# ku222/Attention-GAN

Hardware: AMD Instinct MI355X
Metric: train images/sec at 256×256 stage-3, batch 24/GPU, 1/2/4/8 MI355X (higher is better)
Workload: dtype f32; 1 GPU; full 3-stage AttnGAN 64->128->256 train step: G + 3xD updates + word attention + DAMSM words/sentence loss + KL + 4x fused Adam (BASELINE.json configs[2]); workload_key=full3, batch_per_gpu=24, global_batch=24, gf_dim=32, df_dim=64, emb_dim=256, seq_len=10, text_encoder=bypassed (frozen; N(0,1) embeddings), parallelism=dp1, discriminator_streams=3, launch=eager, gradient_exchange=none (one rank), losses_finite=True

## Files before the change

attention-gan_amd/backend/functional.py:

```python
from __future__ import annotations

import ctypes
import math
from ctypes import byref, c_void_p
from typing import Dict, Optional, Tuple

import contextlib
import os
import weakref

import torch
from torch import Tensor
from torch.autograd import Function
from torch.autograd.function import once_differentiable

from . import lib as L

_PRECISION = [L.PREC_F32]


def set_precision(p: int) -> None:
    if int(p) != _PRECISION[0]:
        for rng in _FLAT_RANGES:
            rng[3], rng[4] = [], None
# ... 418 lines not shown
        return
    cur = torch.cuda.current_stream()
    key = cur.cuda_stream
    if _SIDE_DIRTY.get(key):
        cur.wait_stream(_SIDE_STREAMS[key])
        _SIDE_DIRTY[key] = False


class ActHandoff:
    __slots__ = ("masked",)

    def __init__(self):
        self.masked = False


class _ConvFn(Function):
    @staticmethod
    def forward(ctx, x: Tensor, weight: Tensor, bias: Optional[Tensor], kind: str, cache: Optional[dict], wdst, bdst, act: int = 0,
                handoff_out: Optional[ActHandoff] = None, handoff_in: Optional[ActHandoff] = None):
        x = _act(x, "conv input")
        w = _dev(weight.detach(), "conv weight")
        B, Cin, H, W = x.shape
        Cout, Cin_w, kh, kw = w.shape
        if Cin != Cin_w or kh != kw:
            raise L.AganError(f"conv: input has {Cin} channels, weight {tuple(w.shape)}")
        gf, pf, gd, pd, (OH, OW) = conv_geoms(kind, B, Cin, H, W, Cout, kh)
        pe = effective_precision(gf)
        x, odt = _gather_types(gf, pe, x, get_activation_storage())
        out = torch.empty((B, Cout, OH, OW), dtype=_TORCH_OF[odt], device=x.device)
        b = _dev(bias.detach(), "conv bias") if bias is not None else None
        need_xs = pe == L.PREC_F16X3 or (ctx.needs_input_grad[1] and _needs_amax() and wgrad_effective_precision(gf, pf) == L.PREC_F16X3)
        xs = amax_of(x) if need_xs else None
        _gather(x, packed_weight(w, pf, cache, pe), b, gf, out, kind, "fwd", act, None, pe, xs)
        ctx.x_scale = xs
        if act == L.ACT_NONE:
            ctx.save_for_backward(x, w)
        else:
            ctx.save_for_backward(x, w, out)
        ctx.kind, ctx.has_bias, ctx.cache, ctx.wdst, ctx.bdst, ctx.act = kind, bias is not None, cache, wdst, bdst, act
        ctx.handoff_out = handoff_out if act != L.ACT_NONE else None
        ctx.handoff_in = handoff_in if (handoff_in is not None and Cin > 4) else None
        return out

    @staticmethod
    @once_differentiable
    def backward(ctx, dy: Tensor):
        x, w = ctx.saved_tensors[:2]
        dy = _act(dy, "conv grad")
# ... 43 lines not shown
                if obs is not None:
                    obs.end()
            if want_b:
                dbbuf, bacc, db = _grad_out(ctx.bdst, (Cout,), x)
                L.call("agan_bias_grad", _p(_dev(dy, "conv grad")), _p(dbbuf), B, Cout, dy.shape[2] * dy.shape[3], bacc, _stream())
        if ctx.needs_input_grad[0]:
            dyg, ddt = _gather_types(gd, pe_d, dy, _dt(x))
            dx = torch.empty(x.shape, dtype=_TORCH_OF[ddt], device=x.device)
            mask = x if ctx.handoff_in is not None else None
            if mask is not None and mask.dtype != dx.dtype:
                mask = mask.to(dx.dtype)
            _gather(dyg, packed_weight(w, pd, ctx.cache, pe_d), None, gd, dx, ctx.kind, "dgrad", L.ACT_NONE, mask, pe_d,
                    dys if pe_d == L.PREC_F16X3 else None)
            if mask is not None:
                ctx.handoff_in.masked = True
        return dx, dw, db, None, None, None, None, None, None, None


def conv_fuses_activation(act: int, cout: int) -> bool:
    return act == L.ACT_LRELU and cout > 4


def conv2d(x: Tensor, weight: Tensor, bias: Optional[Tensor] = None, kind: str = "same", cache: Optional[dict] = None,
           wdst=None, bdst=None, act: int = 0, handoff_out: Optional[ActHandoff] = None,
           handoff_in: Optional[ActHandoff] = None) -> Tensor:
    return _ConvFn.apply(x, weight, bias, kind, cache, wdst, bdst, act, handoff_out, handoff_in)


def linear(x: Tensor, weight: Tensor, bias: Optional[Tensor] = None, cache: Optional[dict] = None, wdst=None, bdst=None) -> Tensor:
    B, Cin = x.shape
    y = _ConvFn.apply(x.reshape(B, Cin, 1, 1), weight.view(weight.shape[0], Cin, 1, 1), bias, "same", cache, wdst, bdst)
    return y.view(B, weight.shape[0])


_BN_GROUPS = [1]


@contextlib.contextmanager
def bn_groups(groups: int):
    old = _BN_GROUPS[0]
    _BN_GROUPS[0] = int(groups)
    try:
        yield
    finally:
        _BN_GROUPS[0] = old


class _BnActFn(Function):
    @staticmethod
    def forward(ctx, x, gamma, beta, residual, running_mean, running_var, nbt, training, act, eps, momentum, gdst, bdst, groups):
        x = _act(x, "bn input")
        shape = x.shape
        B, C = shape[0], shape[1]
        HW = x.numel() // (B * C)
        if not training:
            groups = 1
        if B % groups:
            raise L.AganError(f"BatchNorm: batch {B} does not split into {groups} groups")
        Bg = B // groups
        g, b = _dev(gamma.detach(), "bn weight"), _dev(beta.detach(), "bn bias")
        lib = L.load()
        co = C // 2 if act == L.ACT_GLU else C
        odt = get_activation_storage() if HW > 1 else L.DT_F32
        if x.dtype != torch.float32 and _dt(x) != odt:
            x = x.float()
        xdt = _dt(x)
        out = torch.empty((B, co) + tuple(shape[2:]), dtype=_TORCH_OF[odt], device=x.device)
        res = _act(residual, "bn residual") if residual is not None else None
        if res is not None and res.dtype != out.dtype:
            res = res.to(out.dtype)
        if training:
            mean = torch.empty((groups, C), dtype=torch.float32, device=x.device)
            invstd = torch.empty_like(mean)
            nbytes = lib.agan_bn_train_fwd_ws_bytes(Bg, C, HW)
            ws, wsp = _ws(nbytes, x)
            L.call("agan_bn_train_fwd_dt", _p(x), _p(g), _p(b), _p(res), _p(out), _p(mean), _p(invstd), _p(running_mean),
                   _p(running_var), _p(nbt), B, C, HW, float(eps), float(momentum), act, groups, wsp, nbytes, _stream(),
                   _p(_amax_out(out)), xdt, odt)
        else:
            mean = running_mean
            invstd = torch.rsqrt(running_var + eps)
            L.call("agan_bn_act_fwd_dt", _p(x), _p(mean), _p(invstd), _p(g), _p(b), _p(res), _p(out), B, C, HW, act, _stream(),
                   _p(_amax_out(out)), xdt, odt)
        ctx.save_for_backward(x, g, b, mean, invstd)
        ctx.odt = odt
        ctx.act, ctx.training, ctx.has_res, ctx.gdst, ctx.bdst, ctx.groups = act, training, residual is not None, gdst, bdst, groups
        return out

    @staticmethod
    @once_differentiable
    def backward(ctx, dout):
        if not ctx.training:
            raise L.AganError("BatchNorm backward in eval mode is not on the training path")
# ... 3 lines not shown
            dout = dout.to(_TORCH_OF[ctx.odt])
        B, C = x.shape[0], x.shape[1]
        HW = x.numel() // (B * C)
        groups = ctx.groups
        Bg = B // groups
        dx = torch.empty_like(x)
        dgbuf, gacc, dg = _grad_out(ctx.gdst if ctx.needs_input_grad[1] else None, g.shape, x)
        dbbuf, bacc, db = _grad_out(ctx.bdst if ctx.needs_input_grad[2] else None, b.shape, x)
        if gacc != bacc:
            raise L.AganError("BatchNorm weight/bias gradient destinations out of step")
        nbytes = L.load().agan_bn_act_bwd_ws_bytes(Bg, C, HW)
        ws, wsp = _ws(nbytes, x)
        L.call("agan_bn_act_bwd_dt", _p(x), _p(dout), _p(mean), _p(invstd), _p(g), _p(b), _p(dx), _p(dgbuf), _p(dbbuf), B, C, HW,
               ctx.act, gacc, groups, wsp, nbytes, _stream(), _p(_amax_out(dx)), _dt(x), ctx.odt)
        dres = dout if ctx.has_res else None
        return dx, dg, db, dres, None, None, None, None, None, None, None, None, None, None


def bn_act(x, gamma, beta, running_mean, running_var, nbt, training: bool, act: int, residual=None,
           eps: float = 1e-5, momentum: float = 0.1) -> Tensor:
    return _BnActFn.apply(x, gamma, beta, residual, running_mean, running_var, nbt, training, act, eps, momentum,
                          grad_dst(gamma), grad_dst(beta), _BN_GROUPS[0])


class _ActFn(Function):
    @staticmethod
    def forward(ctx, x, act):
        x = _dev(x, "activation input")
        out = torch.empty_like(x)
        L.call("agan_act_fwd", _p(x), _p(out), x.numel(), act, _stream())
        ctx.save_for_backward(out)
        ctx.act = act
        return out

    @staticmethod
    @once_differentiable
    def backward(ctx, dout):
# ... 688 lines not shown
```

attention-gan_amd/backend/lib.py:

```python
from __future__ import annotations

import ctypes
import os
from ctypes import POINTER, Structure, c_char_p, c_double, c_float, c_int, c_int32, c_int64, c_size_t, c_void_p

_HERE = os.path.dirname(os.path.abspath(__file__))
LIB_PATH = os.environ.get("AGAN_LIB") or os.path.join(os.path.dirname(_HERE), "csrc", "libagan_hip.so")

PREC_F32, PREC_BF16, PREC_BF16X3, PREC_F16, PREC_BF16X6, PREC_F16X3 = 0, 1, 2, 3, 4, 5
PRECISIONS = {"f32": PREC_F32, "bf16": PREC_BF16, "bf16x3": PREC_BF16X3, "f16": PREC_F16, "bf16x6": PREC_BF16X6, "f16x3": PREC_F16X3}
PACK_FWD, PACK_DGRAD_S1, PACK_DGRAD_4x4S2, PACK_UP_FWD, PACK_UP_DGRAD, PACK_DGRAD_3x3S2 = 0, 1, 2, 3, 4, 5
ACT_NONE, ACT_GLU, ACT_LRELU, ACT_TANH, ACT_SIGMOID, ACT_RELU = 0, 1, 2, 3, 4, 5
COMM_ID_BYTES = 128
DT_F32, DT_BF16, DT_F16 = 0, 1, 2
AMAX_SLOT = 256
ABI_VERSION = 101


class ConvGeom(Structure):
    _fields_ = [("B", c_int32), ("Cin", c_int32), ("IH", c_int32), ("IW", c_int32),
                ("Cout", c_int32), ("OH", c_int32), ("OW", c_int32), ("R", c_int32), ("S", c_int32),
                ("OS", c_int32), ("SY", c_int32), ("DY", c_int32), ("OY", c_int32 * 2)]


# ... 30 lines not shown
    "agan_pack_weight": (c_int, [_P, _P, c_int, c_int, c_int, c_int, c_int, c_int, _P]),
    "agan_conv_effective_prec": (c_int, [POINTER(ConvGeom), c_int]),
    "agan_conv_wgrad_effective_prec": (c_int, [POINTER(ConvGeom), c_int, c_int]),
    "agan_conv_executed_fraction": (c_double, [POINTER(ConvGeom), c_int, c_int, c_int]),
    "agan_conv_gather_ws_bytes": (c_size_t, [POINTER(ConvGeom), c_int]),
    "agan_conv_ktable_elems": (c_size_t, [POINTER(ConvGeom)]),
    "agan_conv_ktable": (c_int, [POINTER(ConvGeom), _P, _P]),
    "agan_conv_gather": (c_int, [_P, _P, _P, _P, POINTER(ConvGeom), _P, c_int, c_int, _P, _P, c_size_t, _P, _P, _P]),
    "agan_conv_gather_dt": (c_int, [_P, _P, _P, _P, POINTER(ConvGeom), _P, c_int, c_int, _P, _P, c_size_t, _P, _P, _P, c_int, c_int]),
    "agan_conv_gather_dt_supported": (c_int, [POINTER(ConvGeom), c_int, c_int, c_int]),
    "agan_conv_wgrad_dt_supported": (c_int, [POINTER(ConvGeom), c_int, c_int, c_int, c_int]),
    "agan_conv_wgrad_dt": (c_int, [_P, _P, _P, POINTER(ConvGeom), _P, c_int, c_int, c_int, c_int, c_int, _P, c_size_t, _P, _P, _P, c_int, c_int]),
    "agan_bn_stats_dt": (c_int, [_P, c_int, c_int, c_int, c_float, _P, _P, _P, _P, _P, c_float, _P, c_size_t, _P, c_int]),
    "agan_bn_act_fwd_dt": (c_int, [_P, _P, _P, _P, _P, _P, _P, c_int, c_int, c_int, c_int, _P, _P, c_int, c_int]),
    "agan_bn_train_fwd_dt": (c_int, [_P, _P, _P, _P, _P, _P, _P, _P, _P, _P, c_int, c_int, c_int, c_float, c_float, c_int, c_int, _P, c_size_t, _P, _P, c_int, c_int]),
    "agan_bn_act_bwd_dt": (c_int, [_P, _P, _P, _P, _P, _P, _P, _P, _P, c_int, c_int, c_int, c_int, c_int, c_int, _P, c_size_t, _P, _P, c_int, c_int]),
    "agan_absmax": (c_int, [_P, c_size_t, _P, _P]),
    "agan_conv_wgrad_ws_bytes": (c_size_t, [POINTER(ConvGeom)]),
    "agan_conv_wgrad": (c_int, [_P, _P, _P, POINTER(ConvGeom), _P, c_int, c_int, c_int, c_int, c_int, _P, c_size_t, _P, _P, _P]),
    "agan_bias_grad": (c_int, [_P, _P, c_int, c_int, c_int, c_int, _P]),
    "agan_bn_stats_ws_bytes": (c_size_t, [c_int, c_int, c_int]),
    "agan_bn_stats": (c_int, [_P, c_int, c_int, c_int, c_float, _P, _P, _P, _P, _P, c_float, _P, c_size_t, _P]),
    "agan_bn_train_fwd_ws_bytes": (c_size_t, [c_int, c_int, c_int]),
    "agan_bn_train_fwd": (c_int, [_P] * 10 + [c_int, c_int, c_int, c_float, c_float, c_int, c_int, _P, c_size_t, _P, _P]),
    "agan_bn_act_fwd": (c_int, [_P, _P, _P, _P, _P, _P, _P, c_int, c_int, c_int, c_int, _P, _P]),
    "agan_bn_act_bwd_ws_bytes": (c_size_t, [c_int, c_int, c_int]),
    "agan_bn_act_bwd": (c_int, [_P] * 9 + [c_int, c_int, c_int, c_int, c_int, c_int, _P, c_size_t, _P, _P]),
    "agan_act_fwd": (c_int, [_P, _P, c_size_t, c_int, _P]),
    "agan_act_bwd": (c_int, [_P, _P, _P, c_size_t, c_int, _P]),
    "agan_glu_fwd": (c_int, [_P, _P, c_int, c_int, c_int, _P]),
# ... 84 lines not shown
```

attention-gan_amd/csrc/agan_common.h:

```cpp
#pragma once
#include <hip/hip_runtime.h>
#include <stdint.h>
#include <stdio.h>
#include <string.h>

#include "../../include/agan.h"

namespace agan {

constexpr int kWave = 64;

void set_error(const char* fmt, ...);

#define AGAN_REQUIRE(cond, ...)            \
    do {                                    \
        if (!(cond)) {                      \
            agan::set_error(__VA_ARGS__);   \
            return AGAN_EINVAL;             \
        }                                   \
    } while (0)

inline int check_launch(const char* what) {
    hipError_t e = hipGetLastError();
    if (e != hipSuccess) {
// ... 158 lines not shown
}

template <int NT>
__device__ __forceinline__ float block_sum(float v, float* smem) {
    v = wave_sum(v);
    const int w = threadIdx.x >> 6;
    __syncthreads();
    if ((threadIdx.x & 63) == 0) smem[w] = v;
    __syncthreads();
    float r = 0.f;
#pragma unroll
    for (int i = 0; i < NT / 64; ++i) r += smem[i];
    return r;
}

}
```

attention-gan_amd/csrc/bn_act.hip:

```cpp
#include "agan_common.h"

#include <algorithm>
#include <type_traits>

using namespace agan;

namespace {

constexpr float kSlope = 0.2f;

__device__ __forceinline__ float sigmoidf_(float v) { return 1.f / (1.f + __expf(-v)); }

__host__ __device__ __forceinline__ int vec_width(bool any16, int HW) { return (any16 && (HW & 7) == 0) ? 8 : ((HW & 3) == 0 ? 4 : 1); }

constexpr int kLogCap = 64;
thread_local int g_log[kLogCap];
thread_local int g_log_n = 0;
enum { kLogStatsPartial = 1, kLogStatsFinal, kLogStatsRows, kLogFwdApply, kLogSmallFwd, kLogSmallBwd, kLogBwdPartial, kLogBwdFinal,
       kLogBwdApply, kLogActFwd, kLogActBwd, kLogGluFwd, kLogGluBwd };
inline void log_reset() { g_log_n = 0; }
inline void log_launch(int kind, int act, int xdt, int odt, int width) {
    if (g_log_n < kLogCap) g_log[g_log_n] = kind * 100000 + act * 10000 + xdt * 1000 + odt * 100 + width;
    ++g_log_n;
}

struct Chunk { int beg, end; };

__device__ __forceinline__ Chunk chunk_of(int n, int nchunk, int chunk) {
    int len = (cdiv(n, nchunk) + 7) & ~7;
    Chunk c;
    c.beg = min(n, chunk * len);
    c.end = min(n, c.beg + len);
    return c;
}
// ... 355 lines not shown

constexpr int kSmallN = 8192;
constexpr int kSmallPer = kSmallN / 256;

__device__ __forceinline__ void block_sum2_d(double& a, double& b, double (*red)[4]) {
    a = wave_sum_d(a);
    b = wave_sum_d(b);
    const int w = threadIdx.x >> 6;
    __syncthreads();
    if ((threadIdx.x & 63) == 0) { red[0][w] = a; red[1][w] = b; }
    __syncthreads();
    a = red[0][0] + red[0][1] + red[0][2] + red[0][3];
    b = red[1][0] + red[1][1] + red[1][2] + red[1][3];
}

template <int ACT, int XDT, int ODT, int PER = kSmallPer>
__global__ __launch_bounds__(256) void bn_small_fwd_kernel(const void* __restrict__ x, const float* __restrict__ gamma, const float* __restrict__ beta,
                                                           const void* __restrict__ res, void* __restrict__ out, float* __restrict__ mean,
                                                           float* __restrict__ invstd, float* __restrict__ rmean, float* __restrict__ rvar,
                                                           int64_t* __restrict__ nbt, int B, int C, int HW, float eps, float momentum,
                                                           float* __restrict__ amax) {
    __shared__ double red[2][4];
    constexpr bool GLU = ACT == AGAN_ACT_GLU;
    const int Co = GLU ? C / 2 : C;
    const int c = blockIdx.x, n = B * HW;
    if (c == 0 && threadIdx.x == 0 && nbt) *nbt += 1;
    float va[PER], vg[GLU ? PER : 1];
    double s = 0.0, q = 0.0, sg = 0.0, qg = 0.0;
#pragma unroll
    for (int j = 0; j < PER; ++j) {
        const int i = threadIdx.x + j * 256;
        va[j] = 0.f;
        if (GLU) vg[j] = 0.f;
        if (i < n) {
            const int b = i / HW, p = i - b * HW;
            const size_t xi = ((size_t)b * C + c) * HW + p;
            va[j] = ld1<XDT>(x, xi);
            s += va[j];
            q += (double)va[j] * va[j];
            if (GLU) {
                vg[j] = ld1<XDT>(x, xi + (size_t)Co * HW);
                sg += vg[j];
                qg += (double)vg[j] * vg[j];
            }
        }
    }
    block_sum2_d(s, q, red);
    const double m = s / n;
    double var = q / n - m * m;
    var = var < 0.0 ? 0.0 : var;
    const float is = (float)(1.0 / sqrt(var + (double)eps));
    float mgf = 0.f, isg = 0.f;
    double mg = 0.0, varg = 0.0;
    if (GLU) {
        block_sum2_d(sg, qg, red);
        mg = sg / n;
// ... 9 lines not shown
        if (rmean) {
            rmean[c] = (float)((1.0 - momentum) * rmean[c] + momentum * m);
            rvar[c] = (float)((1.0 - momentum) * rvar[c] + momentum * var * ub);
        }
        if (GLU) {
            mean[c + Co] = mgf;
            invstd[c + Co] = isg;
            if (rmean) {
                rmean[c + Co] = (float)((1.0 - momentum) * rmean[c + Co] + momentum * mg);
                rvar[c + Co] = (float)((1.0 - momentum) * rvar[c + Co] + momentum * varg * ub);
            }
        }
    }
    const Affine a = make_affine((float)m, is, gamma[c], beta[c]);
    const Affine g = GLU ? make_affine(mgf, isg, gamma[c + Co], beta[c + Co]) : a;
    float mx = 0.f;
#pragma unroll
    for (int j = 0; j < PER; ++j) {
        const int i = threadIdx.x + j * 256;
        if (i < n) {
            const int b = i / HW, p = i - b * HW;
            const size_t oi = ((size_t)b * Co + c) * HW + p;
            float z = norm_of(a, va[j]);
            if (GLU) z *= sigmoidf_(norm_of(g, vg[j]));
            else if (ACT == AGAN_ACT_LRELU) z = z > 0.f ? z : z * kSlope;
            if (!GLU && ACT == AGAN_ACT_NONE && res) z += ld1<ODT>(res, oi);
            st1<ODT>(out, oi, z);
            mx = fmaxf(mx, fabsf(z));
        }
    }
    if (amax) amax_commit(mx, amax);
}

template <int ACT, int XDT, int ODT, int PER = kSmallPer>
__global__ __launch_bounds__(256) void bn_small_bwd_kernel(const void* __restrict__ x, const void* __restrict__ dout, const float* __restrict__ mean,
                                                           const float* __restrict__ invstd, const float* __restrict__ gamma,
                                                           const float* __restrict__ beta, void* __restrict__ dx, float* __restrict__ dgamma,
                                                           float* __restrict__ dbeta, int B, int C, int HW, int accumulate,
                                                           float* __restrict__ amax) {
    __shared__ double red[2][4];
    constexpr bool GLU = ACT == AGAN_ACT_GLU;
    const int Co = GLU ? C / 2 : C;
    const int c = blockIdx.x, n = B * HW;
    const Affine a = affine_of(mean, invstd, gamma, beta, c);
// ... 352 lines not shown
        if (int e = bn_stats_impl(xg, Bg, C, HW, eps, mg, ig, running_mean, running_var, nbt, momentum, ws, ws_bytes, stream, x_dtype)) return e;
        if (int e = bn_act_fwd_impl(xg, mg, ig, gamma, beta, residual ? off(residual, (size_t)gi * Bg * Co * HW, out_dtype) : nullptr,
                                       off(out, (size_t)gi * Bg * Co * HW, out_dtype), Bg, C, HW, act, stream, out_amax, x_dtype, out_dtype))
            return e;
    }
    return AGAN_OK;
}
int agan_bn_train_fwd(const float* x, const float* gamma, const float* beta, const float* residual, float* out, float* mean,
                      float* invstd, float* running_mean, float* running_var, int64_t* nbt, int B, int C, int HW, float eps,
                      float momentum, int act, int groups, void* ws, size_t ws_bytes, void* stream, float* out_amax) {
    return agan_bn_train_fwd_dt(x, gamma, beta, residual, out, mean, invstd, running_mean, running_var, nbt, B, C, HW, eps, momentum, act,
                                groups, ws, ws_bytes, stream, out_amax, AGAN_DT_F32, AGAN_DT_F32);
}

}
```

attention-gan_amd/csrc/conv.hip:

```cpp
#include "conv_common.h"

#include <cxxabi.h>
#include <cstdlib>


using namespace agan;

using namespace agan::conv;

namespace {

__global__ __launch_bounds__(256) void ktable_kernel(int2* __restrict__ tab, int n, int K, int RS, int S, int IHW, int IW, int DY) {
    const int k = blockIdx.x * 256 + threadIdx.x;
    if (k >= n) return;
    int2 a, b;
    if (k < K) {
        const int c = k / RS, rs = k - c * RS, r = rs / S, q = rs - r * S;
        const int dy = r * DY, dx = q * DY;
        a.x = c * IHW + dy * IW + dx;
        a.y = (dy & 0xFFFF) | (dx << 16);
        b.x = c * IHW * 4;
        b.y = rs * kTapRowBytes;
    } else {
        a.x = 0;
// ... 1053 lines not shown

int agan_conv_ktable(const agan_conv_geom* gg, int32_t* table, void* stream) {
    if (int e = check_geom(gg)) return e;
    AGAN_REQUIRE(table != nullptr, "conv_ktable: null pointer");
    const Geom g = make_geom(gg);
    const int n = ktable_entries(g.K);
    AGAN_LAUNCH(ktable_kernel, dim3(cdiv(n, 256)), dim3(256), 0, as_stream(stream), reinterpret_cast<int2*>(table), n, g.K, g.RS,
                       g.S, g.IH * g.IW, g.IW, g.DY);
    return check_launch("conv_ktable");
}

int agan_conv_gather_dt_supported(const agan_conv_geom* gg, int prec, int in_dtype, int out_dtype) {
    return route_gather(gg, prec, in_dtype, out_dtype, false).path != GatherPath::none ? 1 : 0;
}

int agan_conv_gather_dt(const void* in_v, const void* wkv, const float* bias, void* out_v, const agan_conv_geom* gg, const int32_t* ktable,
                        int prec, int act, const void* lrelu_mask_v, void* ws, size_t ws_bytes, void* stream, const float* in_scale,
                        float* out_amax, int in_dtype, int out_dtype) {
    if (int e = check_geom(gg)) return e;
    AGAN_REQUIRE(in_v && wkv && out_v && ktable, "conv_gather: null pointer");
    AGAN_REQUIRE(act == AGAN_ACT_NONE || (act == AGAN_ACT_LRELU && gg->Cout > 4),
                 "conv_gather: fused activation %d not available for this call (MFMA paths, LeakyReLU only)", act);
    AGAN_REQUIRE(!lrelu_mask_v || (gg->Cout > 4 && act == AGAN_ACT_NONE),
                 "conv_gather: the LeakyReLU-derivative mask needs an MFMA path and no other activation");
    AGAN_REQUIRE(prec == AGAN_PREC_F32 || prec_planes(prec) > 0, "conv_gather: unknown precision mode %d", prec);
    const GatherRoute r = route_gather(gg, prec, in_dtype, out_dtype, bias || act != AGAN_ACT_NONE || lrelu_mask_v);
    AGAN_REQUIRE(r.mode == prec,
                 "conv_gather: precision mode %d does not take this geometry (agan_conv_effective_prec says which one does)", prec);
    AGAN_REQUIRE(r.path != GatherPath::none,
                 "conv_gather: 16-bit activation storage (%d -> %d) is not available for this geometry / precision %d "
                 "(agan_conv_gather_dt_supported)", in_dtype, out_dtype, prec);
    AGAN_REQUIRE(prec != AGAN_PREC_F16X3 || in_scale != nullptr, "conv_gather: AGAN_PREC_F16X3 needs the operand's agan_absmax_scale pair");
    if (int e = check_ws("conv_gather", r.ws_bytes, ws, ws_bytes)) return e;
    const Geom g = make_geom(gg);
    hipStream_t st = as_stream(stream);
    const float* in = static_cast<const float*>(in_v);
    const float* wk = static_cast<const float*>(wkv);
    const float* lrelu_mask = static_cast<const float*>(lrelu_mask_v);
    void* dst = r.split > 1 ? ws : out_v;
    const float* slabs = static_cast<const float*>(ws);
    size_t slab = 0;
    float* sum_amax = nullptr;
    int e = AGAN_OK;
    switch (r.path) {
        case GatherPath::p16:
            slab = r.p16.slab;
            e = launch_main(st, r.split, "conv_gather/p16", [&] {
                launch_p16_gather(in_v, wkv, bias, dst, g, r.p16, prec, act, lrelu_mask_v, st, in_dtype != AGAN_DT_F32, out_dtype != AGAN_DT_F32);
            });
            break;
// ... 11 lines not shown
            break;
        case GatherPath::small_n:
            e = launch_main(st, r.split, "conv_gather/small_n", [&] { launch_gather_small_n(in_v, wk, bias, static_cast<float*>(out_v), g, st, in_dtype); });
            break;
        default: {
            const GatherPlan& p = r.direct;
            slab = p.slab;
            const int2* ktab = reinterpret_cast<const int2*>(ktable);
            e = launch_main(st, r.split, "conv_gather", [&] {
                if (p.bn == 128) launch_gather<128, 2, 2>(in, wk, bias, dst, ktab, g, p, act, lrelu_mask_v, st, out_dtype);
                else if (p.bn == 64) launch_gather<64, 2, 2>(in, wk, bias, dst, ktab, g, p, act, lrelu_mask_v, st, out_dtype);
                else launch_gather<32, 4, 1>(in, wk, bias, dst, ktab, g, p, act, lrelu_mask_v, st, out_dtype);
            });
        }
    }
    if (e || r.split == 1) return e;
    launch_sum_slabs(slabs, r.split, (size_t)g.B * g.Cout * g.OH * g.OW, slab, bias, g.Cout, g.OH * g.OW, out_v, 0, act, lrelu_mask_v, sum_amax, st,
                     out_dtype);
    return check_launch("conv_gather/sum_slabs");
}

int agan_conv_gather(const float* in, const void* wkv, const float* bias, float* out, const agan_conv_geom* gg, const int32_t* ktable,
                     int prec, int act, const float* lrelu_mask, void* ws, size_t ws_bytes, void* stream, const float* in_scale,
                     float* out_amax) {
    return agan_conv_gather_dt(in, wkv, bias, out, gg, ktable, prec, act, lrelu_mask, ws, ws_bytes, stream, in_scale, out_amax,
                               AGAN_DT_F32, AGAN_DT_F32);
}

static const int kPrecs[] = {AGAN_PREC_F32, AGAN_PREC_BF16, AGAN_PREC_BF16X3, AGAN_PREC_F16, AGAN_PREC_BF16X6, AGAN_PREC_F16X3};

size_t agan_conv_wgrad_ws_bytes(const agan_conv_geom* g) {
    if (check_geom(g)) return 0;
    const int pack_mode = g->OS == 2 ? AGAN_PACK_UP_FWD : AGAN_PACK_FWD;
    size_t a = 0;
    for (int prec : kPrecs)
// ... 231 lines not shown
```

attention-gan_amd/utilities/layers.py:

```python
from __future__ import annotations

from math import floor
from typing import List, Optional, Sequence

import torch
from torch import Tensor, nn

from ..backend import functional as HF
from ..backend import lib as L


class HipConv2d(nn.Conv2d):

    def __init__(self, cin: int, cout: int, k: int, stride: int, pad: int, bias: bool, kind: Optional[str] = None):
        super().__init__(cin, cout, kernel_size=k, stride=stride, padding=pad, bias=bias)
        if kind is None:
            if stride == 1 and pad == (k - 1) // 2 and k % 2 == 1:
                kind = "same"
            elif stride == 2 and k == 4 and pad == 1:
                kind = "down"
            else:
                raise NotImplementedError(f"conv k={k} s={stride} p={pad} is not on the AttnGAN hot path")
        self.kind = kind
        self._packed = {}

    def forward(self, x: Tensor, act: int = L.ACT_NONE, handoff_out=None, handoff_in=None) -> Tensor:
        return HF.conv2d(x, self.weight, self.bias, self.kind, self._packed, HF.grad_dst(self.weight),
                         HF.grad_dst(self.bias) if self.bias is not None else None, act, handoff_out, handoff_in)


class HipLinear(nn.Linear):
    def __init__(self, *args, **kwargs):
        super().__init__(*args, **kwargs)
        self._packed = {}

    def forward(self, x: Tensor) -> Tensor:
        return HF.linear(x, self.weight, self.bias, self._packed, HF.grad_dst(self.weight),
                         HF.grad_dst(self.bias) if self.bias is not None else None)


class _BNState:

    def fused(self, x: Tensor, act: int, residual: Optional[Tensor] = None) -> Tensor:
        if self.momentum is None or not self.track_running_stats or not self.affine:
            raise NotImplementedError("only the default BatchNorm configuration is on the hot path")
        return HF.bn_act(x, self.weight, self.bias, self.running_mean, self.running_var, self.num_batches_tracked,
                         self.training, act, residual, self.eps, self.momentum)


class HipBatchNorm2d(nn.BatchNorm2d, _BNState):
    def forward(self, x: Tensor) -> Tensor:
        return self.fused(x, L.ACT_NONE)


class HipBatchNorm1d(nn.BatchNorm1d, _BNState):
    def forward(self, x: Tensor) -> Tensor:
        return self.fused(x, L.ACT_NONE)


class GLU(nn.Module):

    def forward(self, x: Tensor) -> Tensor:
# ... 18 lines not shown
        self.add_module(str(conv_idx), conv)
        if bn_idx is not None:
            self.add_module(str(bn_idx), HipBatchNorm2d(conv.out_channels))
        self._stages.append(_Stage(str(conv_idx), None if bn_idx is None else str(bn_idx), act))
        return self

    def run(self, x: Tensor, residual: Optional[Tensor] = None) -> Tensor:
        last = len(self._stages) - 1
        handoff = None
        for i, st in enumerate(self._stages):
            conv = getattr(self, st.conv)
            if st.bn is None and HF.conv_fuses_activation(st.act, conv.out_channels):
                handoff = HF.ActHandoff() if i < last else None
                x = conv(x, st.act, handoff, None)
                continue
            y = conv(x, L.ACT_NONE, None, handoff)
            handoff = None
            if st.bn is not None:
                x = getattr(self, st.bn).fused(y, st.act, residual if i == last else None)
            elif st.act != L.ACT_NONE:
                x = HF.activation(y, st.act)
            else:
                x = y
        return x

    def forward(self, x: Tensor) -> Tensor:
        return self.run(x)


class _ReluChain(FusedChain):
    def forward(self, x: Tensor) -> Tensor:
        return torch.relu(self.run(x))


# ... 80 lines not shown
```

include/agan.h:

```cpp
#ifndef AGAN_H_
#define AGAN_H_

#include <stddef.h>
#include <stdint.h>

#ifdef __cplusplus
extern "C" {
#endif

#define AGAN_VERSION 101

enum {
    AGAN_OK = 0,
    AGAN_EINVAL = -1,
    AGAN_EWORKSPACE = -2,
    AGAN_ELAUNCH = -3
};

enum {
    AGAN_PREC_F32 = 0,
    AGAN_PREC_BF16 = 1,
    AGAN_PREC_BF16X3 = 2,
    AGAN_PREC_F16 = 3,
    AGAN_PREC_BF16X6 = 4,
// ... 89 lines not shown
int agan_bn_act_fwd_dt(const void* x, const float* mean, const float* invstd, const float* gamma, const float* beta,
                       const void* residual, void* out, int B, int C, int HW, int act, void* stream, float* out_amax, int x_dtype,
                       int out_dtype);
int agan_bn_train_fwd_dt(const void* x, const float* gamma, const float* beta, const void* residual, void* out, float* mean,
                         float* invstd, float* running_mean, float* running_var, int64_t* num_batches_tracked, int B, int C, int HW,
                         float eps, float momentum, int act, int groups, void* ws, size_t ws_bytes, void* stream, float* out_amax,
                         int x_dtype, int out_dtype);
int agan_bn_act_bwd_dt(const void* x, const void* dout, const float* mean, const float* invstd, const float* gamma,
                       const float* beta, void* dx, float* dgamma, float* dbeta, int B, int C, int HW, int act, int accumulate,
                       int groups, void* ws, size_t ws_bytes, void* stream, float* dx_amax, int x_dtype, int out_dtype);
int agan_act_fwd(const float* x, float* out, size_t n, int act, void* stream);
int agan_act_bwd(const float* out, const float* dout, float* dx, size_t n, int act, void* stream);
int agan_glu_fwd(const float* x, float* out, int B, int C, int HW, void* stream);
int agan_glu_bwd(const float* x, const float* dout, float* dx, int B, int C, int HW, void* stream);
int agan_bn_last_launch(int* codes, int capacity);

int agan_attn_fwd(const float* images, const float* words, const float* w, const int64_t* mask, float scale,
                  float* proj, float* ctx, float* attn, int B, int C, int E, int T, int HW, void* stream);
size_t agan_attn_bwd_ws_bytes(int B, int C, int T, int HW);
int agan_attn_bwd(const float* images, const float* words, const float* w, const float* proj, const float* attn,
                  const float* dctx, const float* dattn, float scale, float* dimages, float* dwords, float* dw,
                  int B, int C, int E, int T, int HW, int accumulate, void* ws, size_t ws_bytes, void* stream);
int agan_attn_fwd_dt(const void* images, const float* words, const float* w, const int64_t* mask, float scale, float* proj,
                     void* ctx, float* attn, int B, int C, int E, int T, int HW, void* stream, int dtype);
int agan_attn_bwd_dt(const void* images, const float* words, const float* w, const float* proj, const float* attn,
                     const void* dctx, const float* dattn, float scale, void* dimages, float* dwords, float* dw, int B, int C,
                     int E, int T, int HW, int accumulate, void* ws, size_t ws_bytes, void* stream, int dtype);

int agan_func_attention_fwd(const float* query, const float* context, float gamma1, float scale, float* wctx, float* attn,
                            int B, int D, int L, int S, void* stream);
// ... 97 lines not shown
```

Measured before the change: 987.1 images/s.

## Fuse conv split-K slab reduction into training BatchNorm forward

Conv forward followed by training BatchNorm now defers the conv launch through a handoff object, so the BN step can call a combined conv+BN entry point. When the conv uses split-K slabs and the BN fits the small single-block path, the slab summation, bias add, storing of the conv output and the BN statistics/apply run in one kernel. This removes a separate sum_slabs launch and a reread of the conv output. It adds deferred-execution state that must be flushed on mismatches, which raises correctness risk if the handoff is not consumed.

```diff
diff --git a/attention-gan_amd/backend/functional.py b/attention-gan_amd/backend/functional.py
--- a/attention-gan_amd/backend/functional.py
+++ b/attention-gan_amd/backend/functional.py
@@ -456,10 +456,33 @@
         self.masked = False
 
 
+class BnHandoff:
+    __slots__ = ("pending",)
+
+    def __init__(self):
+        self.pending = None
+
+    def flush(self) -> None:
+        if self.pending is not None:
+            x, wk, b, g, out, kind, pe, xs = self.pending
+            self.pending = None
+            _gather(x, wk, b, g, out, kind, "fwd", L.ACT_NONE, None, pe, xs)
+
+
+_BN_FUSE = [True]
+
+
+def set_bn_fusion(flag: bool) -> bool:
+    old = _BN_FUSE[0]
+    _BN_FUSE[0] = bool(flag)
+    return old
+
+
 class _ConvFn(Function):
     @staticmethod
     def forward(ctx, x: Tensor, weight: Tensor, bias: Optional[Tensor], kind: str, cache: Optional[dict], wdst, bdst, act: int = 0,
-                handoff_out: Optional[ActHandoff] = None, handoff_in: Optional[ActHandoff] = None):
+                handoff_out: Optional[ActHandoff] = None, handoff_in: Optional[ActHandoff] = None,
+                bn_handoff: Optional[BnHandoff] = None):
         x = _act(x, "conv input")
         w = _dev(weight.detach(), "conv weight")
         B, Cin, H, W = x.shape
@@ -473,7 +496,11 @@
         b = _dev(bias.detach(), "conv bias") if bias is not None else None
         need_xs = pe == L.PREC_F16X3 or (ctx.needs_input_grad[1] and _needs_amax() and wgrad_effective_precision(gf, pf) == L.PREC_F16X3)
         xs = amax_of(x) if need_xs else None
-        _gather(x, packed_weight(w, pf, cache, pe), b, gf, out, kind, "fwd", act, None, pe, xs)
+        fuse_bn = bn_handoff is not None and _BN_FUSE[0] and act == L.ACT_NONE and not (_needs_amax() and out.numel() >= _AMAX_FUSE_MIN)
+        if fuse_bn:
+            bn_handoff.pending = (x, packed_weight(w, pf, cache, pe), b, gf, out, kind, pe, xs)
+        else:
+            _gather(x, packed_weight(w, pf, cache, pe), b, gf, out, kind, "fwd", act, None, pe, xs)
         ctx.x_scale = xs
         if act == L.ACT_NONE:
             ctx.save_for_backward(x, w)
@@ -547,7 +574,7 @@
                     dys if pe_d == L.PREC_F16X3 else None)
             if mask is not None:
                 ctx.handoff_in.masked = True
-        return dx, dw, db, None, None, None, None, None, None, None
+        return dx, dw, db, None, None, None, None, None, None, None, None
 
 
 def conv_fuses_activation(act: int, cout: int) -> bool:
@@ -556,8 +583,8 @@
 
 def conv2d(x: Tensor, weight: Tensor, bias: Optional[Tensor] = None, kind: str = "same", cache: Optional[dict] = None,
            wdst=None, bdst=None, act: int = 0, handoff_out: Optional[ActHandoff] = None,
-           handoff_in: Optional[ActHandoff] = None) -> Tensor:
-    return _ConvFn.apply(x, weight, bias, kind, cache, wdst, bdst, act, handoff_out, handoff_in)
+           handoff_in: Optional[ActHandoff] = None, bn_handoff: Optional[BnHandoff] = None) -> Tensor:
+    return _ConvFn.apply(x, weight, bias, kind, cache, wdst, bdst, act, handoff_out, handoff_in, bn_handoff)
 
 
 def linear(x: Tensor, weight: Tensor, bias: Optional[Tensor] = None, cache: Optional[dict] = None, wdst=None, bdst=None) -> Tensor:
@@ -581,7 +608,12 @@
 
 class _BnActFn(Function):
     @staticmethod
-    def forward(ctx, x, gamma, beta, residual, running_mean, running_var, nbt, training, act, eps, momentum, gdst, bdst, groups):
+    def forward(ctx, x, gamma, beta, residual, running_mean, running_var, nbt, training, act, eps, momentum, gdst, bdst, groups,
+                handoff=None):
+        pend = handoff.pending if handoff is not None else None
+        if pend is not None and not (training and pend[4] is x):
+            handoff.flush()
+            pend = None
         x = _act(x, "bn input")
         shape = x.shape
         B, C = shape[0], shape[1]
@@ -596,6 +628,9 @@
         co = C // 2 if act == L.ACT_GLU else C
         odt = get_activation_storage() if HW > 1 else L.DT_F32
         if x.dtype != torch.float32 and _dt(x) != odt:
+            if pend is not None:
+                handoff.flush()
+                pend = None
             x = x.float()
         xdt = _dt(x)
         out = torch.empty((B, co) + tuple(shape[2:]), dtype=_TORCH_OF[odt], device=x.device)
@@ -605,11 +640,25 @@
         if training:
             mean = torch.empty((groups, C), dtype=torch.float32, device=x.device)
             invstd = torch.empty_like(mean)
-            nbytes = lib.agan_bn_train_fwd_ws_bytes(Bg, C, HW)
-            ws, wsp = _ws(nbytes, x)
-            L.call("agan_bn_train_fwd_dt", _p(x), _p(g), _p(b), _p(res), _p(out), _p(mean), _p(invstd), _p(running_mean),
-                   _p(running_var), _p(nbt), B, C, HW, float(eps), float(momentum), act, groups, wsp, nbytes, _stream(),
-                   _p(_amax_out(out)), xdt, odt)
+            if pend is not None:
+                handoff.pending = None
+                xin, wk, cb, cg, _, kind, pe, xs = pend
+                nbytes = lib.agan_conv_bn_train_fwd_ws_bytes(byref(cg), pe, groups)
+                ws, wsp = _ws(nbytes, xin)
+                obs = _OBSERVER[0]
+                if obs is not None:
+                    obs.begin(kind, "fwd", cg, xin.element_size(), x.element_size())
+                L.call("agan_conv_bn_train_fwd_dt", _p(xin), _p(wk), _p(cb), _p(x), byref(cg), _p(ktable(cg, x.device)), pe, _p(xs),
+                       _p(g), _p(b), _p(res), _p(out), _p(mean), _p(invstd), _p(running_mean), _p(running_var), _p(nbt), float(eps),
+                       float(momentum), act, groups, wsp, nbytes, _stream(), _p(_amax_out(out)), _dt(xin), xdt, odt)
+                if obs is not None:
+                    obs.end()
+            else:
+                nbytes = lib.agan_bn_train_fwd_ws_bytes(Bg, C, HW)
+                ws, wsp = _ws(nbytes, x)
+                L.call("agan_bn_train_fwd_dt", _p(x), _p(g), _p(b), _p(res), _p(out), _p(mean), _p(invstd), _p(running_mean),
+                       _p(running_var), _p(nbt), B, C, HW, float(eps), float(momentum), act, groups, wsp, nbytes, _stream(),
+                       _p(_amax_out(out)), xdt, odt)
         else:
             mean = running_mean
             invstd = torch.rsqrt(running_var + eps)
@@ -643,13 +692,13 @@
         L.call("agan_bn_act_bwd_dt", _p(x), _p(dout), _p(mean), _p(invstd), _p(g), _p(b), _p(dx), _p(dgbuf), _p(dbbuf), B, C, HW,
                ctx.act, gacc, groups, wsp, nbytes, _stream(), _p(_amax_out(dx)), _dt(x), ctx.odt)
         dres = dout if ctx.has_res else None
-        return dx, dg, db, dres, None, None, None, None, None, None, None, None, None, None
+        return dx, dg, db, dres, None, None, None, None, None, None, None, None, None, None, None
 
 
 def bn_act(x, gamma, beta, running_mean, running_var, nbt, training: bool, act: int, residual=None,
-           eps: float = 1e-5, momentum: float = 0.1) -> Tensor:
+           eps: float = 1e-5, momentum: float = 0.1, handoff: Optional[BnHandoff] = None) -> Tensor:
     return _BnActFn.apply(x, gamma, beta, residual, running_mean, running_var, nbt, training, act, eps, momentum,
-                          grad_dst(gamma), grad_dst(beta), _BN_GROUPS[0])
+                          grad_dst(gamma), grad_dst(beta), _BN_GROUPS[0], handoff)
 
 
 class _ActFn(Function):
diff --git a/attention-gan_amd/backend/lib.py b/attention-gan_amd/backend/lib.py
--- a/attention-gan_amd/backend/lib.py
+++ b/attention-gan_amd/backend/lib.py
@@ -68,6 +68,9 @@
     "agan_bn_stats_dt": (c_int, [_P, c_int, c_int, c_int, c_float, _P, _P, _P, _P, _P, c_float, _P, c_size_t, _P, c_int]),
     "agan_bn_act_fwd_dt": (c_int, [_P, _P, _P, _P, _P, _P, _P, c_int, c_int, c_int, c_int, _P, _P, c_int, c_int]),
     "agan_bn_train_fwd_dt": (c_int, [_P, _P, _P, _P, _P, _P, _P, _P, _P, _P, c_int, c_int, c_int, c_float, c_float, c_int, c_int, _P, c_size_t, _P, _P, c_int, c_int]),
+    "agan_conv_bn_train_fwd_ws_bytes": (c_size_t, [POINTER(ConvGeom), c_int, c_int]),
+    "agan_conv_bn_train_fwd_dt": (c_int, [_P, _P, _P, _P, POINTER(ConvGeom), _P, c_int, _P, _P, _P, _P, _P, _P, _P, _P, _P, _P, c_float, c_float,
+                                          c_int, c_int, _P, c_size_t, _P, _P, c_int, c_int, c_int]),
     "agan_bn_act_bwd_dt": (c_int, [_P, _P, _P, _P, _P, _P, _P, _P, _P, c_int, c_int, c_int, c_int, c_int, c_int, _P, c_size_t, _P, _P, c_int, c_int]),
     "agan_absmax": (c_int, [_P, c_size_t, _P, _P]),
     "agan_conv_wgrad_ws_bytes": (c_size_t, [POINTER(ConvGeom)]),
diff --git a/attention-gan_amd/csrc/agan_common.h b/attention-gan_amd/csrc/agan_common.h
--- a/attention-gan_amd/csrc/agan_common.h
+++ b/attention-gan_amd/csrc/agan_common.h
@@ -196,4 +196,10 @@
     return r;
 }
 
-}
+bool bn_small_fits(int B, int HW);
+int bn_small_slab_fwd(const float* slabs, int nsplit, size_t slab, const float* bias, void* xout, const float* gamma, const float* beta,
+                      const void* residual, void* out, float* mean, float* invstd, float* running_mean, float* running_var, int64_t* nbt,
+                      int B, int C, int HW, float eps, float momentum, int act, int groups, hipStream_t st, float* out_amax, int x_dtype,
+                      int out_dtype);
+
+}
diff --git a/attention-gan_amd/csrc/bn_act.hip b/attention-gan_amd/csrc/bn_act.hip
--- a/attention-gan_amd/csrc/bn_act.hip
+++ b/attention-gan_amd/csrc/bn_act.hip
@@ -17,7 +17,7 @@
 thread_local int g_log[kLogCap];
 thread_local int g_log_n = 0;
 enum { kLogStatsPartial = 1, kLogStatsFinal, kLogStatsRows, kLogFwdApply, kLogSmallFwd, kLogSmallBwd, kLogBwdPartial, kLogBwdFinal,
-       kLogBwdApply, kLogActFwd, kLogActBwd, kLogGluFwd, kLogGluBwd };
+       kLogBwdApply, kLogActFwd, kLogActBwd, kLogGluFwd, kLogGluBwd, kLogSlabFwd };
 inline void log_reset() { g_log_n = 0; }
 inline void log_launch(int kind, int act, int xdt, int odt, int width) {
     if (g_log_n < kLogCap) g_log[g_log_n] = kind * 100000 + act * 10000 + xdt * 1000 + odt * 100 + width;
@@ -403,17 +403,14 @@
     b = red[1][0] + red[1][1] + red[1][2] + red[1][3];
 }
 
-template <int ACT, int XDT, int ODT, int PER = kSmallPer>
-__global__ __launch_bounds__(256) void bn_small_fwd_kernel(const void* __restrict__ x, const float* __restrict__ gamma, const float* __restrict__ beta,
-                                                           const void* __restrict__ res, void* __restrict__ out, float* __restrict__ mean,
-                                                           float* __restrict__ invstd, float* __restrict__ rmean, float* __restrict__ rvar,
-                                                           int64_t* __restrict__ nbt, int B, int C, int HW, float eps, float momentum,
-                                                           float* __restrict__ amax) {
-    __shared__ double red[2][4];
+template <int ACT, int ODT, int PER, class Load>
+__device__ __forceinline__ void bn_small_fwd_body(Load&& load, const float* __restrict__ gamma, const float* __restrict__ beta,
+                                                  const void* __restrict__ res, void* __restrict__ out, float* __restrict__ mean,
+                                                  float* __restrict__ invstd, float* __restrict__ rmean, float* __restrict__ rvar,
+                                                  int B, int C, int HW, float eps, float momentum, float& mx, double (*red)[4]) {
     constexpr bool GLU = ACT == AGAN_ACT_GLU;
     const int Co = GLU ? C / 2 : C;
     const int c = blockIdx.x, n = B * HW;
-    if (c == 0 && threadIdx.x == 0 && nbt) *nbt += 1;
     float va[PER], vg[GLU ? PER : 1];
     double s = 0.0, q = 0.0, sg = 0.0, qg = 0.0;
 #pragma unroll
@@ -423,12 +420,11 @@
         if (GLU) vg[j] = 0.f;
         if (i < n) {
             const int b = i / HW, p = i - b * HW;
-            const size_t xi = ((size_t)b * C + c) * HW + p;
-            va[j] = ld1<XDT>(x, xi);
+            va[j] = load(b, p, 0);
             s += va[j];
             q += (double)va[j] * va[j];
             if (GLU) {
-                vg[j] = ld1<XDT>(x, xi + (size_t)Co * HW);
+                vg[j] = load(b, p, 1);
                 sg += vg[j];
                 qg += (double)vg[j] * vg[j];
             }
@@ -468,7 +464,6 @@
     }
     const Affine a = make_affine((float)m, is, gamma[c], beta[c]);
     const Affine g = GLU ? make_affine(mgf, isg, gamma[c + Co], beta[c + Co]) : a;
-    float mx = 0.f;
 #pragma unroll
     for (int j = 0; j < PER; ++j) {
         const int i = threadIdx.x + j * 256;
@@ -482,6 +477,82 @@
             st1<ODT>(out, oi, z);
             mx = fmaxf(mx, fabsf(z));
         }
+    }
+}
+
+template <int ACT, int XDT, int ODT, int PER = kSmallPer>
+__global__ __launch_bounds__(256) void bn_small_fwd_kernel(const void* __restrict__ x, const float* __restrict__ gamma, const float* __restrict__ beta,
+                                                           const void* __restrict__ res, void* __restrict__ out, float* __restrict__ mean,
+                                                           float* __restrict__ invstd, float* __restrict__ rmean, float* __restrict__ rvar,
+                                                           int64_t* __restrict__ nbt, int B, int C, int HW, float eps, float momentum,
+                                                           float* __restrict__ amax) {
+    __shared__ double red[2][4];
+    const int Co = ACT == AGAN_ACT_GLU ? C / 2 : C;
+    const int c = blockIdx.x;
+    if (c == 0 && threadIdx.x == 0 && nbt) *nbt += 1;
+    auto load = [&](int b, int p, int half) { return ld1<XDT>(x, ((size_t)b * C + c + half * Co) * HW + p); };
+    float mx = 0.f;
+    bn_small_fwd_body<ACT, ODT, PER>(load, gamma, beta, res, out, mean, invstd, rmean, rvar, B, C, HW, eps, momentum, mx, red);
+    if (amax) amax_commit(mx, amax);
+}
+
+template <bool MANY>
+__device__ __forceinline__ float slab_sum(const float* __restrict__ ws, int nsplit, size_t slab, size_t q, const float* bias) {
+    const float* p = ws + q;
+    float a;
+    if (!MANY) {
+        float v[8];
+#pragma unroll
+        for (int k = 0; k < 8; ++k)
+            if (k < nsplit) v[k] = p[(size_t)k * slab];
+        a = v[0];
+#pragma unroll
+        for (int k = 1; k < 8; ++k)
+            if (k < nsplit) a += v[k];
+    } else {
+        float t[8];
+#pragma unroll
+        for (int grp = 0; grp < 8; ++grp) {
+            float s = 0.f;
+            int sp = grp;
+            for (; sp + 24 < nsplit; sp += 32) {
+                const float v0 = p[(size_t)sp * slab], v1 = p[(size_t)(sp + 8) * slab];
+                const float v2 = p[(size_t)(sp + 16) * slab], v3 = p[(size_t)(sp + 24) * slab];
+                s += (v0 + v1) + (v2 + v3);
+            }
+            for (; sp < nsplit; sp += 8) s += p[(size_t)sp * slab];
+            t[grp] = s;
+        }
+        a = t[0];
+#pragma unroll
+        for (int grp = 1; grp < 8; ++grp) a += t[grp];
+    }
+    return bias ? a + *bias : a;
+}
+
+template <int ACT, int XDT, int ODT, int PER, bool MANY>
+__global__ __launch_bounds__(256) void bn_small_slab_fwd_kernel(const float* __restrict__ ws, int nsplit, size_t slab, const float* __restrict__ bias,
+                                                                void* __restrict__ xout, const float* __restrict__ gamma,
+                                                                const float* __restrict__ beta, const void* __restrict__ res,
+                                                                void* __restrict__ out, float* __restrict__ mean, float* __restrict__ invstd,
+                                                                float* __restrict__ rmean, float* __restrict__ rvar, int64_t* __restrict__ nbt,
+                                                                int groups, int Bg, int C, int HW, float eps, float momentum,
+                                                                float* __restrict__ amax) {
+    __shared__ double red[2][4];
+    const int Co = ACT == AGAN_ACT_GLU ? C / 2 : C;
+    const int c = blockIdx.x;
+    float mx = 0.f;
+    for (int gi = 0; gi < groups; ++gi) {
+        if (c == 0 && threadIdx.x == 0 && nbt) *nbt += 1;
+        auto load = [&](int b, int p, int half) {
+            const size_t q = ((size_t)(gi * Bg + b) * C + c + half * Co) * HW + p;
+            const float v = slab_sum<MANY>(ws, nsplit, slab, q, bias ? bias + c + half * Co : nullptr);
+            st1<XDT>(xout, q, v);
+            return round_dt<XDT>(v);
+        };
+        const size_t go = (size_t)gi * Bg * Co * HW * dt_size(ODT);
+        bn_small_fwd_body<ACT, ODT, PER>(load, gamma, beta, res ? static_cast<const char*>(res) + go : nullptr, static_cast<char*>(out) + go, mean + (size_t)gi * C,
+                                         invstd + (size_t)gi * C, rmean, rvar, Bg, C, HW, eps, momentum, mx, red);
     }
     if (amax) amax_commit(mx, amax);
 }
@@ -864,3 +935,48 @@
 }
 
 }
+
+namespace agan {
+
+bool bn_small_fits(int B, int HW) { return HW > 1 && (long long)B * HW <= kSmallN; }
+
+int bn_small_slab_fwd(const float* slabs, int nsplit, size_t slab, const float* bias, void* xout, const float* gamma, const float* beta,
+                      const void* residual, void* out, float* mean, float* invstd, float* running_mean, float* running_var, int64_t* nbt,
+                      int B, int C, int HW, float eps, float momentum, int act, int groups, hipStream_t st, float* out_amax, int x_dtype,
+                      int out_dtype) {
+    log_reset();
+    AGAN_REQUIRE(slabs && nsplit > 1 && xout && gamma && beta && out && mean && invstd && B > 0 && C > 0, "conv_bn_train_fwd: bad argument");
+    AGAN_REQUIRE(act == AGAN_ACT_NONE || act == AGAN_ACT_GLU || act == AGAN_ACT_LRELU, "conv_bn_train_fwd: activation %d", act);
+    AGAN_REQUIRE(act != AGAN_ACT_GLU || (C % 2 == 0), "channels dont divide 2!");
+    AGAN_REQUIRE(!(residual && act != AGAN_ACT_NONE), "conv_bn_train_fwd: residual only with ACT_NONE");
+    AGAN_REQUIRE((running_mean == nullptr) == (running_var == nullptr), "conv_bn_train_fwd: running_mean/var must come together");
+    AGAN_REQUIRE(groups >= 1 && B % groups == 0, "conv_bn_train_fwd: batch %d does not split into %d groups", B, groups);
+    AGAN_REQUIRE(bn_dt_ok(x_dtype, out_dtype), "conv_bn_train_fwd: storage types %d -> %d", x_dtype, out_dtype);
+    const int Bg = B / groups;
+    AGAN_REQUIRE(bn_small_fits(Bg, HW), "conv_bn_train_fwd: %d x %d values per channel is not a one-launch BatchNorm", Bg, HW);
+    const int Co = act == AGAN_ACT_GLU ? C / 2 : C;
+    for (int gi = 0; gi < groups; ++gi) {
+        const size_t xo = (size_t)gi * Bg * C * HW, oo = (size_t)gi * Bg * Co * HW;
+        const float* sg = slabs + xo;
+        void* xg = static_cast<char*>(xout) + xo * dt_size(x_dtype);
+        const void* rg = residual ? static_cast<const char*>(residual) + oo * dt_size(out_dtype) : nullptr;
+        void* og = static_cast<char*>(out) + oo * dt_size(out_dtype);
+        float* mg = mean + (size_t)gi * C;
+        float* ig = invstd + (size_t)gi * C;
+#define AGAN_LM(A, XD, OD, P, M) hipLaunchKernelGGL((bn_small_slab_fwd_kernel<A, XD, OD, P, M>), dim3(Co), dim3(256), 0, st, sg, nsplit, slab, bias, xg, gamma, beta, rg, og, mg, ig, running_mean, running_var, nbt, 1, Bg, C, HW, eps, momentum, out_amax)
+#define AGAN_LP(A, XD, OD, P) do { log_launch(kLogSlabFwd, A, XD, OD, P); if (nsplit > 8) AGAN_LM(A, XD, OD, P, true); else AGAN_LM(A, XD, OD, P, false); } while (0)
+#define AGAN_L(A, XD, OD) do { if (Bg * HW <= 512) AGAN_LP(A, XD, OD, 2); else if (Bg * HW <= 2048) AGAN_LP(A, XD, OD, 8); else AGAN_LP(A, XD, OD, kSmallPer); } while (0)
+#define AGAN_C(XD, OD)                                           \
+    if (act == AGAN_ACT_GLU) AGAN_L(AGAN_ACT_GLU, XD, OD);       \
+    else if (act == AGAN_ACT_LRELU) AGAN_L(AGAN_ACT_LRELU, XD, OD); \
+    else AGAN_L(AGAN_ACT_NONE, XD, OD);
+        AGAN_BN_DT(x_dtype, out_dtype, AGAN_C);
+#undef AGAN_C
+#undef AGAN_L
+#undef AGAN_LP
+#undef AGAN_LM
+    }
+    return check_launch("conv_bn_train_fwd/slab_bn");
+}
+
+}
diff --git a/attention-gan_amd/csrc/conv.hip b/attention-gan_amd/csrc/conv.hip
--- a/attention-gan_amd/csrc/conv.hip
+++ b/attention-gan_amd/csrc/conv.hip
@@ -1091,9 +1091,18 @@
     return route_gather(gg, prec, in_dtype, out_dtype, false).path != GatherPath::none ? 1 : 0;
 }
 
-int agan_conv_gather_dt(const void* in_v, const void* wkv, const float* bias, void* out_v, const agan_conv_geom* gg, const int32_t* ktable,
-                        int prec, int act, const void* lrelu_mask_v, void* ws, size_t ws_bytes, void* stream, const float* in_scale,
-                        float* out_amax, int in_dtype, int out_dtype) {
+}
+
+struct GatherSlabs {
+    const float* slabs = nullptr;
+    size_t slab = 0;
+    int split = 1;
+    float* amax = nullptr;
+};
+
+static int gather_main(const void* in_v, const void* wkv, const float* bias, void* out_v, const agan_conv_geom* gg, const int32_t* ktable,
+                       int prec, int act, const void* lrelu_mask_v, void* ws, size_t ws_bytes, hipStream_t st, const float* in_scale,
+                       float* out_amax, int in_dtype, int out_dtype, GatherSlabs& gs) {
     if (int e = check_geom(gg)) return e;
     AGAN_REQUIRE(in_v && wkv && out_v && ktable, "conv_gather: null pointer");
     AGAN_REQUIRE(act == AGAN_ACT_NONE || (act == AGAN_ACT_LRELU && gg->Cout > 4),
@@ -1110,7 +1119,6 @@
     AGAN_REQUIRE(prec != AGAN_PREC_F16X3 || in_scale != nullptr, "conv_gather: AGAN_PREC_F16X3 needs the operand's agan_absmax_scale pair");
     if (int e = check_ws("conv_gather", r.ws_bytes, ws, ws_bytes)) return e;
     const Geom g = make_geom(gg);
-    hipStream_t st = as_stream(stream);
     const float* in = static_cast<const float*>(in_v);
     const float* wk = static_cast<const float*>(wkv);
     const float* lrelu_mask = static_cast<const float*>(lrelu_mask_v);
@@ -1152,11 +1160,60 @@
             });
         }
     }
-    if (e || r.split == 1) return e;
-    launch_sum_slabs(slabs, r.split, (size_t)g.B * g.Cout * g.OH * g.OW, slab, bias, g.Cout, g.OH * g.OW, out_v, 0, act, lrelu_mask_v, sum_amax, st,
-                     out_dtype);
+    gs.slabs = slabs;
+    gs.slab = slab;
+    gs.split = r.split;
+    gs.amax = sum_amax;
+    return e;
+}
+
+extern "C" {
+
+int agan_conv_gather_dt(const void* in_v, const void* wkv, const float* bias, void* out_v, const agan_conv_geom* gg, const int32_t* ktable,
+                        int prec, int act, const void* lrelu_mask_v, void* ws, size_t ws_bytes, void* stream, const float* in_scale,
+                        float* out_amax, int in_dtype, int out_dtype) {
+    hipStream_t st = as_stream(stream);
+    GatherSlabs gs;
+    if (int e = gather_main(in_v, wkv, bias, out_v, gg, ktable, prec, act, lrelu_mask_v, ws, ws_bytes, st, in_scale, out_amax, in_dtype, out_dtype, gs))
+        return e;
+    if (gs.split == 1) return AGAN_OK;
+    launch_sum_slabs(gs.slabs, gs.split, (size_t)gg->B * gg->Cout * gg->OH * gg->OW, gs.slab, bias, gg->Cout, gg->OH * gg->OW, out_v, 0, act,
+                     lrelu_mask_v, gs.amax, st, out_dtype);
     return check_launch("conv_gather/sum_slabs");
 }
+
+size_t agan_conv_bn_train_fwd_ws_bytes(const agan_conv_geom* g, int prec, int groups) {
+    if (check_geom(g) || groups < 1 || g->B % groups) return 0;
+    return std::max(agan_conv_gather_ws_bytes(g, prec), agan_bn_train_fwd_ws_bytes(g->B / groups, g->Cout, g->OH * g->OW));
+}
+
+int agan_conv_bn_train_fwd_dt(const void* in, const void* wk, const float* bias, void* conv_out, const agan_conv_geom* g, const int32_t* ktable,
+                              int prec, const float* in_scale, const float* gamma, const float* beta, const void* residual, void* out,
+                              float* mean, float* invstd, float* running_mean, float* running_var, int64_t* num_batches_tracked, float eps,
+                              float momentum, int act, int groups, void* ws, size_t ws_bytes, void* stream, float* out_amax, int in_dtype,
+                              int conv_dtype, int out_dtype) {
+    if (int e = check_geom(g)) return e;
+    AGAN_REQUIRE(groups >= 1 && g->B % groups == 0, "conv_bn_train_fwd: batch %d does not split into %d groups", g->B, groups);
+    if (int e = check_ws("conv_bn_train_fwd", agan_conv_bn_train_fwd_ws_bytes(g, prec, groups), ws, ws_bytes)) return e;
+    hipStream_t st = as_stream(stream);
+    const int HW = g->OH * g->OW;
+    GatherSlabs gs;
+    if (int e = gather_main(in, wk, bias, conv_out, g, ktable, prec, AGAN_ACT_NONE, nullptr, ws, ws_bytes, st, in_scale, nullptr, in_dtype,
+                            conv_dtype, gs))
+        return e;
+    if (gs.split > 1 && bn_small_fits(g->B / groups, HW) && HW % 4 == 0)
+        return bn_small_slab_fwd(gs.slabs, gs.split, gs.slab, bias, conv_out, gamma, beta, residual, out, mean, invstd, running_mean,
+                                 running_var, num_batches_tracked, g->B, g->Cout, HW, eps, momentum, act, groups, st, out_amax, conv_dtype,
+                                 out_dtype);
+    if (gs.split > 1) {
+        launch_sum_slabs(gs.slabs, gs.split, (size_t)g->B * g->Cout * HW, gs.slab, bias, g->Cout, HW, conv_out, 0, AGAN_ACT_NONE, nullptr, nullptr,
+                         st, conv_dtype);
+        if (int e = check_launch("conv_bn_train_fwd/sum_slabs")) return e;
+    }
+    return agan_bn_train_fwd_dt(conv_out, gamma, beta, residual, out, mean, invstd, running_mean, running_var, num_batches_tracked, g->B,
+                                g->Cout, HW, eps, momentum, act, groups, ws, ws_bytes, stream, out_amax, conv_dtype, out_dtype);
+}
+
 
 int agan_conv_gather(const float* in, const void* wkv, const float* bias, float* out, const agan_conv_geom* gg, const int32_t* ktable,
                      int prec, int act, const float* lrelu_mask, void* ws, size_t ws_bytes, void* stream, const float* in_scale,
diff --git a/attention-gan_amd/utilities/layers.py b/attention-gan_amd/utilities/layers.py
--- a/attention-gan_amd/utilities/layers.py
+++ b/attention-gan_amd/utilities/layers.py
@@ -24,9 +24,9 @@
         self.kind = kind
         self._packed = {}
 
-    def forward(self, x: Tensor, act: int = L.ACT_NONE, handoff_out=None, handoff_in=None) -> Tensor:
+    def forward(self, x: Tensor, act: int = L.ACT_NONE, handoff_out=None, handoff_in=None, bn_handoff=None) -> Tensor:
         return HF.conv2d(x, self.weight, self.bias, self.kind, self._packed, HF.grad_dst(self.weight),
-                         HF.grad_dst(self.bias) if self.bias is not None else None, act, handoff_out, handoff_in)
+                         HF.grad_dst(self.bias) if self.bias is not None else None, act, handoff_out, handoff_in, bn_handoff)
 
 
 class HipLinear(nn.Linear):
@@ -41,11 +41,11 @@
 
 class _BNState:
 
-    def fused(self, x: Tensor, act: int, residual: Optional[Tensor] = None) -> Tensor:
+    def fused(self, x: Tensor, act: int, residual: Optional[Tensor] = None, handoff=None) -> Tensor:
         if self.momentum is None or not self.track_running_stats or not self.affine:
             raise NotImplementedError("only the default BatchNorm configuration is on the hot path")
         return HF.bn_act(x, self.weight, self.bias, self.running_mean, self.running_var, self.num_batches_tracked,
-                         self.training, act, residual, self.eps, self.momentum)
+                         self.training, act, residual, self.eps, self.momentum, handoff)
 
 
 class HipBatchNorm2d(nn.BatchNorm2d, _BNState):
@@ -94,10 +94,12 @@
                 handoff = HF.ActHandoff() if i < last else None
                 x = conv(x, st.act, handoff, None)
                 continue
-            y = conv(x, L.ACT_NONE, None, handoff)
+            bn = getattr(self, st.bn) if st.bn is not None else None
+            bh = HF.BnHandoff() if bn is not None and bn.training else None
+            y = conv(x, L.ACT_NONE, None, handoff, bh)
             handoff = None
-            if st.bn is not None:
-                x = getattr(self, st.bn).fused(y, st.act, residual if i == last else None)
+            if bn is not None:
+                x = bn.fused(y, st.act, residual if i == last else None, bh)
             elif st.act != L.ACT_NONE:
                 x = HF.activation(y, st.act)
             else:
diff --git a/include/agan.h b/include/agan.h
--- a/include/agan.h
+++ b/include/agan.h
@@ -127,6 +127,12 @@
 int agan_glu_fwd(const float* x, float* out, int B, int C, int HW, void* stream);
 int agan_glu_bwd(const float* x, const float* dout, float* dx, int B, int C, int HW, void* stream);
 int agan_bn_last_launch(int* codes, int capacity);
+size_t agan_conv_bn_train_fwd_ws_bytes(const agan_conv_geom* g, int prec, int groups);
+int agan_conv_bn_train_fwd_dt(const void* in, const void* wk, const float* bias, void* conv_out, const agan_conv_geom* g,
+                              const int32_t* ktable, int prec, const float* in_scale, const float* gamma, const float* beta,
+                              const void* residual, void* out, float* mean, float* invstd, float* running_mean, float* running_var,
+                              int64_t* num_batches_tracked, float eps, float momentum, int act, int groups, void* ws, size_t ws_bytes,
+                              void* stream, float* out_amax, int in_dtype, int conv_dtype, int out_dtype);
 
 int agan_attn_fwd(const float* images, const float* words, const float* w, const int64_t* mask, float scale,
                   float* proj, float* ctx, float* attn, int B, int C, int E, int T, int HW, void* stream);
```

Result: no change. 984.4 images/s, median of 2 (-0.3%).
